# CleanDiffuserTeam/CleanDiffuser

Hardware: AMD Instinct MI355X
Metric: denoised trajectories/sec @ (B=256,H=32,D=23) 20-step DDIM (higher is better)
Workload: dtype f32; 1 GPU; BASELINE configs[1]: JannerUNet1d Diffuser H=32 D=23, 20-step DDIM, global B=256, whole DiscreteDiffusionSDE.sample() call as a pipeline makes it (initial draw inside); batch_per_gpu=256, global_batch=256, horizon=32, dim=23, sample_steps=20, world_size=1, parallelism=batch-sharded x1; the only data-path collective is the all-gather of the result

## Files before the change

### cleandiffuser_amd/csrc/cdx_unet2.hip

```cpp
#include <hip/hip_runtime.h>
#include <stdint.h>
#include <string.h>

#include "../../include/cdx.h"
#include "cdx_ops2.h"

typedef float f32x4 __attribute__((ext_vector_type(4)));
typedef const int __attribute__((address_space(4))) cint;
#pragma clang diagnostic push
#pragma clang diagnostic ignored "-Wold-style-cast"
static __device__ __forceinline__ const cint* as_const(const int* p) { return (const cint*)p; }
#pragma clang diagnostic pop

void cdx_set_err(const char* msg);

template <int NWV> struct WG {
    static constexpr int THREADS = NWV * 64;
    static constexpr int PF = NWV == 8 ? 8 : 16;
    static constexpr int OPW = CDX2_HDR_WORDS + NWV * CDX2_ITEM_WORDS;
};

namespace {

__device__ __forceinline__ float mish2(float x) {
// ... 100 lines not shown
__device__ __forceinline__ int load_desc(const int* __restrict__ ops, int op, int lane, int wave) {
    const int w = lane < CDX2_HDR_WORDS ? lane : CDX2_HDR_WORDS + wave * CDX2_ITEM_WORDS + (lane & (CDX2_ITEM_WORDS - 1));
    return ops[op * WG<NWV>::OPW + w];
}
__device__ __forceinline__ Item inline_item(int vd) {
    const int b = CDX2_HDR_WORDS;
    return make_item(CDX2_DW(vd, b + CDX2_I2_WOFF), CDX2_DW(vd, b + CDX2_I2_NQ), CDX2_DW(vd, b + CDX2_I2_TAPCC),
                     CDX2_DW(vd, b + CDX2_I2_PART), CDX2_DW(vd, b + CDX2_I2_COL0), CDX2_DW(vd, b + CDX2_I2_PADOOFF),
                     CDX2_DW(vd, b + CDX2_I2_SRCSTR), CDX2_DW(vd, b + CDX2_I2_CCN));
}

__device__ __forceinline__ void stamp(unsigned long long* slot, int tid) {
    if (slot && tid == 0) *slot = __builtin_amdgcn_s_memtime();
}

typedef unsigned u32x4 __attribute__((ext_vector_type(4)));
#ifndef CDX2_WPOLICY
#define CDX2_WPOLICY 0
#endif
#ifndef CDX2_PARAMS_ALL
#define CDX2_PARAMS_ALL 0
#endif
#define CDX2_N_CUS 256
#define CDX2_GETREG_XCC_ID ((3 << 11) | 20)
#ifndef CDX2_XCHG_FAST
#define CDX2_XCHG_FAST 1
#endif
#ifndef CDX2_XCHG_NOWAIT
#define CDX2_XCHG_NOWAIT 0
#endif
#ifndef CDX2_PROF_FETCH
#define CDX2_PROF_FETCH 0
#endif
#ifndef CDX2_PIPE_PARAMS
#define CDX2_PIPE_PARAMS 1
#endif
#ifndef CDX2_MUL24
#define CDX2_MUL24 1
#endif
static __device__ __forceinline__ int mul24i(int a, int b) { return CDX2_MUL24 ? __mul24(a, b) : a * b; }
static __device__ __forceinline__ int wave_of(int tid) { return __builtin_amdgcn_readfirstlane(tid >> 6); }
#pragma clang diagnostic push
#pragma clang diagnostic ignored "-Wold-style-cast"
struct WStream {
    __amdgpu_buffer_rsrc_t rs;
    int lane16;
    __device__ __forceinline__ WStream(const float* wblob, int lane)
        : rs(__builtin_amdgcn_make_buffer_rsrc((void*)wblob, 0, 0x7fffffff, 0x00020000)), lane16(lane * 16) {}
    __device__ __forceinline__ f32x4 load(int woff, int q) const {
        return __builtin_bit_cast(f32x4, __builtin_amdgcn_raw_buffer_load_b128(rs, lane16, woff * 4 + q * 1024, CDX2_WPOLICY));
    }
};
#pragma clang diagnostic pop

template <int PF> struct Ring { f32x4 rec[PF]; };

template <class M, int NT, int T, int NWV, bool PROF, bool GRP = false>
__device__ __forceinline__ void conv_kloop(const Geom& g, const float* __restrict__ wblob, int vd, const cint* ops,
                                           Item it, int n_items, float* __restrict__ lds, int tf, int lane, int wave,
                                           Ring<WG<NWV>::PF>& ring, unsigned long long* prof, int tune) {
    constexpr int PF = WG<NWV>::PF, NW = NWV;
    constexpr int BD = NWV == 4 ? ((M::KSTEP == 4 && NT * T == 1) ? 8 : 4)
                                : (NT * T == 1 ? (M::KSTEP == 4 ? 8 : 4) : (NT * T == 2 ? 4 : 2));
    constexpr int NA = NWV == 4 ? 4 : ((M::KSTEP == 4 && NT == 1) ? 4 : 2);
    static_assert(PF % BD == 0, "operand ring must divide the weight ring");
    const int ptid = (wave == 0 && lane == 0) ? 0 : 1;
    for (int item = wave; item < n_items; item += NW) {
        if (item != wave) it = load_item(ops + CDX2_DW(vd, CDX2_W2_ITEMS) + (item - NW) * CDX2_ITEM_WORDS);
        const int nq = it.nq, ccn = it.ccn;
        int cc = it.cc;
        int cur[NT], tstep[NT], mcol[NT];
#pragma unroll
        for (int nt = 0; nt < NT; ++nt) {
            mcol[nt] = it.col0 + nt * M::COLS + M::col(lane);
            const bool valid = mcol[nt] < g.l_cols;
            int mrow = mul24i(mcol[nt], g.cstride);
            if (GRP && g.grows) mrow = mul24i(mcol[nt] >> g.gsh, g.grows) + mul24i(mcol[nt] & ((1 << g.gsh) - 1), g.cstride);
            const int row = valid ? mrow - it.pad + CDX2_HALO2 + it.tap : 0;
            cur[nt] = it.src + __mul24(row, it.sstr) + M::koff(lane) + cc * M::KSTEP;
            tstep[nt] = (valid ? it.sstr : 0) - ccn * M::KSTEP;
        }
        if (PROF && !CDX2_PROF_FETCH && prof && item == 0) { asm volatile("" ::"s"(nq), "v"(cur[0])); stamp(prof + 4, ptid); }
        f32x4 acc[T][NT][NA];
#pragma unroll
        for (int t = 0; t < T; ++t)
#pragma unroll
            for (int nt = 0; nt < NT; ++nt)
#pragma unroll
                for (int j = 0; j < NA; ++j) acc[t][nt][j] = (f32x4){0.f, 0.f, 0.f, 0.f};

        const WStream ws(wblob, lane);
        const int woff = it.woff;
#define CDX2_WLOAD(q) ws.load(woff, (q))
// ... 79 lines not shown
#pragma unroll
                        for (int nt = 0; nt < NT; ++nt)
                            bq[ua % BD][t][nt] = *reinterpret_cast<const f32x4*>(
                                ldsb + (ua < PF ? rb[nt] : rbn[nt]) + t * tf * 4 + (ua % PF) * M::KSTEP * 4);
#pragma unroll
                    for (int j = 0; j < 4; ++j)
#pragma unroll
                        for (int t = 0; t < T; ++t)
#pragma unroll
                            for (int nt = 0; nt < NT; ++nt)
                                acc[t][nt][j % NA] = M::mfma(wr[u][j], bq[u % BD][t][nt][j], acc[t][nt][j % NA]);
                    if (u > 0) refill(u - 1, qi + u - 1 + PF);
                    else if (qi > 0) refill(PF - 1, qi - 1 + PF);
                    if (NWV == 4 || T >= 2) __builtin_amdgcn_sched_barrier(0);
                }
#pragma unroll
                for (int nt = 0; nt < NT; ++nt) rb[nt] = rbn[nt];
            }
            cc = cc0 + BD - 2;
#pragma unroll
            for (int nt = 0; nt < NT; ++nt) cur[nt] = rb[nt] / 4 + (BD - 2) * M::KSTEP;
        }
        for (; qi < nq; qi += PF) {
#pragma unroll
            for (int u = 0; u < PF; ++u) {
                if (qi + u >= nq) break;
                chunk(wr[u], u, qi + u + BD - 1 < nq);
                const int q = qi + u - 1 + PF;
                if (q >= PF && q < nq) refill((u + PF - 1) % PF, q);
            }
        }
        if (NWV == 8) __builtin_amdgcn_s_setprio(0);
        if (PROF && !CDX2_PROF_FETCH && prof && item == 0) { asm volatile("" ::"v"(acc[0][0][0][0]), "v"(acc[0][0][1][0])); stamp(prof + 6, ptid); }
#pragma unroll
        for (int t = 0; t < T; ++t)
#pragma unroll
            for (int nt = 0; nt < NT; ++nt) {
                if (mcol[nt] < g.l_cols) {
                    const int n = mul24i(mcol[nt], g.ostride) + it.ooff;
                    f32x4 dd = acc[t][nt][0];
                    if (NA == 2) dd += acc[t][nt][NA - 1];
                    if (NA == 4) dd = (acc[t][nt][0] + acc[t][nt][1]) + (acc[t][nt][NA / 2] + acc[t][nt][NA - 1]);
                    *reinterpret_cast<f32x4*>(lds + t * tf + g.stage + it.part + mul24i(n, g.sstride) + M::drow(lane)) = dd;
                }
            }
    }
}

struct EpiDesc {
    int flags, c_out, l_out, coutp, sstride, ksplit, dst, dstride, res, rstride, shift, nk;
    int save, savestr, stats, dst2, d2stride;
    int kpost;
    float inv_cnt;
    float odiv;
    int cgreal4;
};
template <bool BWD>
__device__ __forceinline__ EpiDesc decode_epi(int vd) {
    EpiDesc e;
    e.flags = CDX2_DW(vd, CDX2_W2_FLAGS); e.c_out = CDX2_DW(vd, CDX2_W2_COUT); e.l_out = CDX2_DW(vd, CDX2_W2_LOUT);
    e.coutp = CDX2_DW(vd, CDX2_W2_COUTP); e.sstride = CDX2_DW(vd, CDX2_W2_SSTRIDE); e.ksplit = CDX2_DW(vd, CDX2_W2_KSPLIT);
    e.dst = CDX2_DW(vd, CDX2_W2_DST); e.dstride = CDX2_DW(vd, CDX2_W2_DST_STRIDE); e.res = CDX2_DW(vd, CDX2_W2_RES);
    e.rstride = CDX2_DW(vd, CDX2_W2_RES_STRIDE); e.shift = CDX2_DW(vd, CDX2_W2_CG4_SHIFT); e.nk = CDX2_DW(vd, CDX2_W2_NK);
    e.inv_cnt = __int_as_float(CDX2_DW(vd, CDX2_W2_INV_CNT));
    e.kpost = CDX2_DW(vd, CDX2_W2_KPOST);
    e.odiv = BWD ? 1.0f : __int_as_float(CDX2_DW(vd, CDX2_W2_ODIV));
    e.cgreal4 = BWD ? 0 : CDX2_DW(vd, CDX2_W2_CGREAL4);
    e.save = e.savestr = e.stats = e.dst2 = e.d2stride = 0;
    if (BWD && (e.flags & (CDX2_F2_SAVE | CDX2_F2_GNBWD))) {
        e.save = CDX2_DW(vd, CDX2_W2_SAVE); e.savestr = CDX2_DW(vd, CDX2_W2_SAVE_STRIDE); e.stats = CDX2_DW(vd, CDX2_W2_STATS);
        e.dst2 = CDX2_DW(vd, CDX2_W2_DST2); e.d2stride = CDX2_DW(vd, CDX2_W2_DST2_STRIDE);
    }
    return e;
}

// ... 232 lines not shown
template <int THREADS>
__device__ __forceinline__ void run_head_fwd(const cdx_unet2_launch& L, int vd, const float* __restrict__ emb_row, float* __restrict__ tl,
                                             int tid, float* __restrict__ out) {
    const int hidden = CDX2_DW(vd, CDX2_W2_COUT), len = CDX2_DW(vd, CDX2_W2_LOUT), ch = CDX2_DW(vd, CDX2_W2_LCOLS);
    const int src = CDX2_DW(vd, CDX2_W2_RES), sstr = CDX2_DW(vd, CDX2_W2_RES_STRIDE);
    const float* __restrict__ w1 = L.wblob + CDX2_DW(vd, CDX2_W2_BOFF);
    const float* __restrict__ w2 = L.wblob + CDX2_DW(vd, CDX2_W2_GAMMA);
    const float* __restrict__ ev = emb_row + CDX2_DW(vd, CDX2_W2_EMB);
    float* hz = tl + L.stage_off;
    for (int j = tid; j < hidden; j += THREADS) {
        float z = ev[j];
        for (int l = 0; l < len; ++l) {
#pragma unroll 8
            for (int c = 0; c < ch; ++c) z = fmaf(w1[(size_t)(l * ch + c) * hidden + j], tl[src + (l + CDX2_HALO2) * sstr + c], z);
        }
        hz[j] = w2[j] * mish2(z);
    }
    __syncthreads();
    if (tid == 0 && out != nullptr) {
        float y = w2[hidden];
        for (int j = 0; j < hidden; ++j) y += hz[j];
        *out = y;
    }
    __syncthreads();
}

template <int PF>
__device__ __forceinline__ void prefetch_ring(const Item& it, const float* __restrict__ wblob, int lane, Ring<PF>& ring) {
    const WStream ws(wblob, lane);
#pragma unroll
    for (int u = 0; u < PF; ++u) ring.rec[u] = ws.load(it.woff, u);
}

template <bool COND, bool SPLIT_T, bool ALL, bool MLP = false, bool GRP = false>
__device__ __forceinline__ EpiParams load_params(const cdx_unet2_launch& L, int vd, const float* __restrict__ emb_row, int emb_tstride,
                                                 int tid, int wave, bool epi_wave) {
    const int etid = tid & 255, li = etid & 31;
    int grp = etid >> 5;
    if (GRP) {
        const int xg = CDX2_DW(vd, CDX2_W2_XG);
        if (xg & CDX2_XG_GOP) grp = (xg & 255) + (grp & ((((xg >> 8) & 255) - (xg & 255)) - 1));
    }
    const int flags = CDX2_DW(vd, CDX2_W2_FLAGS), coutp = CDX2_DW(vd, CDX2_W2_COUTP), shift = CDX2_DW(vd, CDX2_W2_CG4_SHIFT);
    const int c = mul24i(grp, coutp >> 3) + 4 * (li & ((1 << shift) - 1));
    const float* __restrict__ pbi = ((MLP && (flags & CDX2_F2_BIAS_EMB)) ? emb_row : L.wblob) + CDX2_DW(vd, CDX2_W2_BOFF) + c;
    const bool gn = (flags & (CDX2_F2_GN | CDX2_F2_GNBWD)) != 0;
    const float* __restrict__ pem = emb_row + (COND && SPLIT_T ? (wave >> 2) * emb_tstride : 0) + CDX2_DW(vd, CDX2_W2_EMB) + c;
    EpiParams P;
    if (ALL) {
        P.bi = *reinterpret_cast<const f32x4*>(pbi);
        P.pb = *reinterpret_cast<const f32x4*>(CDX2_DW(vd, CDX2_W2_KPOST) ? L.wblob + CDX2_DW(vd, CDX2_W2_PBIAS) + c : pbi);
        P.ga = *reinterpret_cast<const f32x4*>(gn ? L.wblob + CDX2_DW(vd, CDX2_W2_GAMMA) + c : pbi);
        P.be = *reinterpret_cast<const f32x4*>(gn ? L.wblob + CDX2_DW(vd, CDX2_W2_BETA) + c : pbi);
        P.em = *reinterpret_cast<const f32x4*>((flags & CDX2_F2_EMB) ? pem + ((COND && (flags & CDX2_F2_FILM)) ? coutp : 0) : pbi);
        P.sc = P.bi;
        if (COND) P.sc = *reinterpret_cast<const f32x4*>((flags & CDX2_F2_FILM) ? pem : pbi);
        return P;
    }
    P.bi = P.ga = P.be = P.em = P.pb = P.sc = (f32x4){0.f, 0.f, 0.f, 0.f};
    if (epi_wave) {
        P.bi = *reinterpret_cast<const f32x4*>(pbi);
        if (CDX2_DW(vd, CDX2_W2_KPOST)) P.pb = *reinterpret_cast<const f32x4*>(L.wblob + CDX2_DW(vd, CDX2_W2_PBIAS) + c);
        if (gn) {
            P.ga = *reinterpret_cast<const f32x4*>(L.wblob + CDX2_DW(vd, CDX2_W2_GAMMA) + c);
            P.be = *reinterpret_cast<const f32x4*>(L.wblob + CDX2_DW(vd, CDX2_W2_BETA) + c);
        }
        if (COND && (flags & CDX2_F2_FILM)) {
            P.sc = *reinterpret_cast<const f32x4*>(pem);
            P.em = *reinterpret_cast<const f32x4*>(pem + coutp);
        } else if (flags & CDX2_F2_EMB) P.em = *reinterpret_cast<const f32x4*>(pem);
    }
    return P;
}

struct OpFetch {
    EpiParams P;
    int vdn2;
};
template <int T, bool BWD> constexpr bool pipe_params() { return CDX2_PIPE_PARAMS && T < 3 && !BWD; }

struct XState {
    int m, k;
    unsigned seq;
    bool dead;
};

__device__ __forceinline__ void xchg_report(int what, const XState& X, int seq, int item, int grp) {
    const KArg* S0 = kernarg();
    asm volatile("" : "+s"(S0));
    int* e = S0->xerr;
    e[1] = what; e[2] = (int)blockIdx.x; e[3] = seq; e[4] = item;
    e[5] = (int)(__builtin_amdgcn_s_getreg(CDX2_GETREG_XCC_ID) & 15); e[6] = X.m; e[7] = grp;
// ... 97 lines not shown
        int pending = (1 << km1) - 1, spins = 0;
        while (pending) {
#pragma unroll
            for (int r = 0; r < 3; ++r) {
                if (!(pending & (1 << r))) continue;
                if (__float_as_uint(a[r][1]) == seq && __float_as_uint(a[r][3]) == seq && __float_as_uint(b[r][1]) == seq &&
                    __float_as_uint(b[r][3]) == seq) {
                    *reinterpret_cast<f32x4*>(tl + dst + row + cc[r]) = (f32x4){a[r][0], a[r][2], b[r][0], b[r][2]};
                    pending &= ~(1 << r);
                } else {
                    asm volatile("" ::: "memory");
                    const f32x4* src = reinterpret_cast<const f32x4*>(tile + (size_t)(tbase + cc[r]) * 2);
                    a[r] = __builtin_nontemporal_load(src);
                    b[r] = __builtin_nontemporal_load(src + 1);
                }
            }
            if (pending) {
                if (X.dead || ++spins > 200000) {
                    if (!X.dead) xchg_report(1, X, (int)seq, j, grp_idx);
                    X.dead = true;
                    break;
                }
                __builtin_amdgcn_s_sleep(1);
            }
        }
    }
}

template <int T, int NWV, bool BWD, bool PROF, bool COND, bool MLP = false, bool SPLIT = false, bool MEMBER = SPLIT>
__device__ __forceinline__ void run_op(const cdx_unet2_launch& L, const cint* ops, int vd, int vdn, Item& it,
                                       const float* __restrict__ emb_row, int emb_tstride, float* __restrict__ lds, int tid,
                                       Ring<WG<NWV>::PF>& ring, unsigned long long* prof, int b0, OpFetch& F,
                                       const float* __restrict__ emb_next, int emb_next_tstride, int op_next2, int pass = 0,
                                       XState* X = nullptr) {
    constexpr bool SPLIT_T = NWV == 8 && T >= 2;
    constexpr bool PIPE = pipe_params<T, BWD>();
    constexpr bool PARAMS_AFTER_BARRIER = PIPE && T >= 2;
    auto fetch_next = [&](bool params) {
        it = inline_item(vdn);
        if (PROF && CDX2_PROF_FETCH == 1) stamp(prof ? prof + 4 : nullptr, tid);
        if (wave_of(tid) < CDX2_DW(vdn, CDX2_W2_NITEMS)) prefetch_ring(it, L.wblob, tid & 63, ring);
        if (PROF && CDX2_PROF_FETCH == 1) stamp(prof ? prof + 5 : nullptr, tid);
        if (PIPE) {
            if (params)
                F.P = load_params<COND, SPLIT_T, false, MLP, MEMBER>(L, vdn, emb_next, emb_next_tstride, tid, wave_of(tid), NWV == 4 || SPLIT_T || wave_of(tid) < 4);
            if (PROF && CDX2_PROF_FETCH == 1) stamp(prof ? prof + 6 : nullptr, tid);
            F.vdn2 = load_desc<NWV>(L.ops, op_next2 + (MEMBER ? X->m * L.n_ops : 0), tid & 63, wave_of(tid));
        }
    };
    const int lane = tid & 63, wave = __builtin_amdgcn_readfirstlane(tid >> 6);
    const int tf = L.traj_floats;
    if (BWD && CDX2_DW(vd, CDX2_W2_KIND) == CDX2_KIND2_HEAD) {
        fetch_next(true);
#pragma unroll 1
        for (int t = 0; t < T; ++t) run_head<WG<NWV>::THREADS>(L, vd, emb_row, lds + t * tf, tid);
        return;
    }
    if (BWD && CDX2_DW(vd, CDX2_W2_KIND) == CDX2_KIND2_LOADX) {
        fetch_next(true);
        const int dst = CDX2_DW(vd, CDX2_W2_DST), dstr = CDX2_DW(vd, CDX2_W2_DST_STRIDE);
        const int len = CDX2_DW(vd, CDX2_W2_LOUT), ch = CDX2_DW(vd, CDX2_W2_COUT);
        const int b_end = L.traj_first + L.traj_count;
        const KArg* S = kernarg();
        asm volatile("" : "+s"(S));
#pragma unroll 1
        for (int t = 0; t < T; ++t) {
            const float* __restrict__ xg = S->x_out + (size_t)(b0 + t) * len * ch;
            const bool real = b0 + t < b_end;
            for (int i = tid; i < (len + 2 * CDX2_HALO2) * dstr; i += WG<NWV>::THREADS) {
                const int r = i / dstr, c = i - r * dstr, n = r - CDX2_HALO2;
                lds[t * tf + dst + i] = (real && n >= 0 && n < len && c < ch) ? xg[n * ch + c] : 0.f;
            }
        }
        __syncthreads();
        return;
    }
    if (MLP && CDX2_DW(vd, CDX2_W2_KIND) == CDX2_KIND2_LOADC) {
        fetch_next(true);
// ... 5 lines not shown
        asm volatile("" : "+s"(S));
        const float* __restrict__ cg = pass == 0 ? S->ctx : nullptr;
#pragma unroll 1
        for (int t = 0; t < T; ++t) {
            const bool real = cg != nullptr && b0 + t < b_end;
            const float* __restrict__ cb = cg + (size_t)(b0 + t) * len * ch;
            for (int i = tid; i < (len + 2 * CDX2_HALO2) * dstr; i += WG<NWV>::THREADS) {
                const int r = i / dstr, c = i - r * dstr, n = r - CDX2_HALO2;
                lds[t * tf + dst + i] = (real && n >= 0 && n < len && c < ch) ? cb[n * ch + c] : 0.f;
            }
        }
        __syncthreads();
        return;
    }
    const int flags = CDX2_DW(vd, CDX2_W2_FLAGS), coutp = CDX2_DW(vd, CDX2_W2_COUTP), shift = CDX2_DW(vd, CDX2_W2_CG4_SHIFT);
    const int l_out = CDX2_DW(vd, CDX2_W2_LOUT), sstride = CDX2_DW(vd, CDX2_W2_SSTRIDE);
    int gmap0 = 0;
    if (SPLIT && (CDX2_DW(vd, CDX2_W2_XG) & CDX2_XG_GOP)) gmap0 = CDX2_DW(vd, CDX2_W2_GMAP);
    const Geom g{CDX2_DW(vd, CDX2_W2_LCOLS), CDX2_DW(vd, CDX2_W2_CSTRIDE), CDX2_DW(vd, CDX2_W2_OSTRIDE), sstride, L.stage_off,
                 gmap0 & 255, gmap0 >> 8};
    const bool epi_wave = NWV == 4 || SPLIT_T || wave < 4;
    const bool halo_wave = NWV == 4 || SPLIT_T || wave >= 4;

    const int etid = tid & 255;
    const int grp = etid >> 5, li = etid & 31;
    const int c = mul24i(grp, coutp >> 3) + 4 * (li & ((1 << shift) - 1));
    const int pos0 = li >> shift, pstep = 32 >> shift;
    const int nv = (coutp >> 5) * l_out;
    EpiParams P = PIPE ? F.P : load_params<COND, SPLIT_T, CDX2_PARAMS_ALL != 0, MLP, MEMBER>(L, vd, emb_row, emb_tstride, tid, wave, epi_wave);

    const int n_items = CDX2_DW(vd, CDX2_W2_NITEMS);
    if (SPLIT && gmap0 != 0) {
        if (CDX2_DW(vd, CDX2_W2_MODE) == CDX_MODE_4X4) {
            if (CDX2_DW(vd, CDX2_W2_NT) == 1) conv_kloop<M4, 1, T, NWV, PROF, SPLIT>(g, L.wblob, vd, ops, it, n_items, lds, tf, lane, wave, ring, prof, L.tune);
            else conv_kloop<M4, 2, T, NWV, PROF, SPLIT>(g, L.wblob, vd, ops, it, n_items, lds, tf, lane, wave, ring, prof, L.tune);
        } else {
            conv_kloop<M16, 1, T, NWV, PROF, SPLIT>(g, L.wblob, vd, ops, it, n_items, lds, tf, lane, wave, ring, prof, L.tune);
        }
    } else if (CDX2_DW(vd, CDX2_W2_MODE) == CDX_MODE_4X4) {
        if (CDX2_DW(vd, CDX2_W2_NT) == 1) conv_kloop<M4, 1, T, NWV, PROF>(g, L.wblob, vd, ops, it, n_items, lds, tf, lane, wave, ring, prof, L.tune);
        else conv_kloop<M4, 2, T, NWV, PROF>(g, L.wblob, vd, ops, it, n_items, lds, tf, lane, wave, ring, prof, L.tune);
    } else {
        conv_kloop<M16, 1, T, NWV, PROF>(g, L.wblob, vd, ops, it, n_items, lds, tf, lane, wave, ring, prof, L.tune);
    }
    if (PROF) stamp(prof ? prof + 7 : nullptr, tid);
    fetch_next(!PARAMS_AFTER_BARRIER);
    if (PROF) stamp(prof ? prof + 1 : nullptr, tid);
    __syncthreads();
    if (PROF) stamp(prof ? prof + 2 : nullptr, tid);
    const EpiParams Pnext = PARAMS_AFTER_BARRIER ? load_params<COND, SPLIT_T, false, MLP, MEMBER>(L, vdn, emb_next, emb_next_tstride, tid, wave, epi_wave)
                                                 : (PIPE ? F.P : P);

    const EpiDesc e = decode_epi<BWD>(vd);
    int xgw = 0, gmap = 0;
    if (SPLIT) {
        int vde = vd;
        asm volatile("" : "+v"(vde));
        xgw = CDX2_DW(vde, CDX2_W2_XG);
        if (BWD && (e.flags & (CDX2_F2_SAVE | CDX2_F2_GNBWD | CDX2_F2_DUAL))) xgw = 0;
        if (xgw & (CDX2_XG_GOP | CDX2_XG_TRAJ)) gmap = CDX2_DW(vde, CDX2_W2_GMAP);
    }
    if (SPLIT && (xgw & CDX2_XG_GOP)) {
        const int gx_lo = xgw & 255, gpm = ((xgw >> 8) & 255) - gx_lo, grows = gmap >> 8;
        const bool xfast = CDX2_XCHG_FAST && (xgw & CDX2_XG_XCHG) != 0;
        const unsigned xseq = X->seq + 1;
        float* xtile = xfast ? exchange_tile(*X, xseq, __float_as_int(lds[T * tf])) : nullptr;
        if (epi_wave) {
            const int g_t = __builtin_amdgcn_readfirstlane(gpm == 4 ? grp >> 2 : grp >> 1);
            const int cgo = mul24i(gx_lo + (grp & (gpm - 1)), coutp >> 3) + 4 * (li & ((1 << shift) - 1));
            EpiDesc eg = e;
            eg.dst += g_t * grows * e.dstride;
            eg.res += g_t * grows * e.rstride;
            eg.l_out = l_out * X->k;
            const int stage_g = g.stage + g_t * l_out * sstride - gx_lo * (coutp >> 3);
            bool withhold = false;
            if (xfast) {
                const KArg* S0 = kernarg();
                asm volatile("" : "+s"(S0));
                withhold = S0->fault != 0 && X->m == S0->fault - 1;
            }
            const Pub pub{xtile, __uint_as_float(xseq), g_t * l_out, e.coutp, xfast && !withhold};
            if (e.nk == 1) epilogue<1, BWD, COND, MLP, true>(lds, P, eg, stage_g, cgo, pos0, pstep, li, nv, lane, grp, nullptr, &pub);
            else epilogue<2, BWD, COND, MLP, true>(lds, P, eg, stage_g, cgo, pos0, pstep, li, nv, lane, grp, nullptr, &pub);
// ... 149 lines not shown
    __syncthreads();
    auto logp_only_f = [&]() -> bool {
        if (!BWD) return false;
        const KArg* S0 = kernarg();
        asm volatile("" : "+s"(S0));
        return S0->n_steps == 0 && S0->logp_out != nullptr;
    };
    const int n_iter = logp_only_f() ? 0 : (L.n_steps > 0 ? L.n_steps : 1);
    const int HDp = (HD + 3) & ~3;
    constexpr bool PIPE = pipe_params<T, BWD>();
    constexpr bool SPLIT_T0 = NWV == 8 && T >= 2;
    int n_pass_all = 1;
    if (COND) {
        const KArg* S0 = kernarg();
        asm volatile("" : "+s"(S0));
        n_pass_all = S0->n_pass == 2 ? 2 : 1;
    }
    auto emb_of = [&](int step, int pass, int& tstride) -> const float* {
        const float* row = L.emb + (size_t)step * L.emb_ld;
        tstride = 0;
        if (COND) {
            const KArg* S0 = kernarg();
            asm volatile("" : "+s"(S0));
            if (pass == 1) row = S0->emb_u + (size_t)step * L.emb_ld;
            else if (S0->emb_per_traj) {
                row = L.emb + ((size_t)step * L.batch + b0) * L.emb_ld;
                tstride = L.emb_ld;
            }
        }
        return row;
    };
    OpFetch F;
    int vdn_keep = 0;
    if (PIPE) {
        int ts0;
        const float* row0 = emb_of(0, 0, ts0);
        F.P = load_params<COND, SPLIT_T0, false, MLP>(L, vd, row0, ts0, tid, wave, NWV == 4 || SPLIT_T0 || wave < 4);
        vdn_keep = load_desc<NWV>(L.ops, moff + (L.n_ops > 1 ? 1 : 0), lane, wave);
    }
    for (int step = 0; step < n_iter; ++step) {
      const int n_pass = n_pass_all;
#pragma unroll 1
      for (int pass = 0; pass < n_pass; ++pass) {
        int emb_tstride, emb_next_tstride;
        const float* __restrict__ emb_row = emb_of(step, pass, emb_tstride);
        const bool last_fwd = pass + 1 == n_pass && step + 1 >= n_iter;
        const float* __restrict__ emb_fwd_next = last_fwd ? emb_of(step, pass, emb_next_tstride)
                                                          : emb_of(pass + 1 < n_pass ? step : step + 1, pass + 1 < n_pass ? pass + 1 : 0, emb_next_tstride);
        const int ts_fwd_next = emb_next_tstride;
        for (int oi = 0; oi < L.n_ops; ++oi) {
            const int vdn = PIPE ? vdn_keep : load_desc<NWV>(L.ops, moff + (oi + 1 < L.n_ops ? oi + 1 : 0), lane, wave);
            unsigned long long* pslot = (profiling && step == (L.n_steps > 1 ? 1 : 0)) ? lprof + (size_t)oi * 8 : nullptr;
            if (PROF) stamp(pslot, tid);
            const bool wrap = oi + 1 >= L.n_ops;
            int on2 = oi + 2;
            if (on2 >= L.n_ops) on2 -= L.n_ops;
            if (on2 >= L.n_ops) on2 = 0;
            run_op<T, NWV, BWD, PROF, COND, MLP, SPLIT, SPLIT>(L, ops, vd, vdn, it, emb_row, emb_tstride, lds, tid, ring, pslot, b0, F,
                                                               wrap ? emb_fwd_next : emb_row, wrap ? ts_fwd_next : emb_tstride, on2,
                                                               (MLP && n_pass == 1 && step > 0) ? 2 : pass, &X);
            vd = vdn;
            if (PIPE) vdn_keep = F.vdn2;
        }
        if (COND && n_pass == 2 && pass == 0) {
            const KArg* S = kernarg();
            asm volatile("" : "+s"(S));
#pragma unroll 1
            for (int t = 0; t < T; ++t) {
                if (b0 + t >= b_end) break;
                const size_t xbase = (size_t)(b0 + t) * HD;
                float* tl = lds + t * tf;
                float* wsb = S->ws + (size_t)(b0 + t) * S->ws_floats;
                const float c_in = S->edm_plan ? S->steps[step].alpha : 1.0f;
                for (int e = tid; e < HD; e += THREADS) {
                    const int n = e / D, c = e - n * D;
                    wsb[2 * HDp + e] = tl[S->pred_off + n * S->pred_stride + c];
                    if (S->compact) tl[S->x_off + n * S->x_stride + c] = c_in * S->x_out[xbase + e];
                }
                if (S->compact) {
                    const int xs = S->x_stride, xb = S->x_off - CDX2_HALO2 * xs;
                    for (int i = tid; i < (H + 2 * CDX2_HALO2) * xs; i += THREADS) {
                        const int r = i / xs, c = i - r * xs;
                        if (r < CDX2_HALO2 || r >= H + CDX2_HALO2 || c >= D) tl[xb + i] = 0.f;
                    }
                }
            }
            __syncthreads();
        }
      }
        if (L.n_steps == 0) break;
        const KArg* S = kernarg();
        asm volatile("" : "+s"(S));
        const cdx_step st = S->steps[step];
        const float al = st.alpha, sg = st.sigma;
        const float k0 = st.k[0], k1 = st.k[1], k2 = st.k[2], k3 = st.k[3], k4 = st.k[4];
        const bool edm = COND && st.kind >= 5;
        const bool xglob = S->compact || edm;
        const float c_next = (edm && step + 1 < S->n_steps) ? S->steps[step + 1].alpha : 1.0f;
#pragma unroll 1
        for (int t = 0; t < T; ++t) {
            if (b0 + t >= b_end) break;
            const int b = b0 + t;
            const size_t xbase = (size_t)b * HD;
            float* tl = lds + t * tf;
            float* wsb = (COND && (xglob || n_pass == 2)) ? S->ws + (size_t)b * S->ws_floats : nullptr;
            for (int e = tid; e < HD; e += THREADS) {
                const int n = e / D, c = e - n * D;
                const int xo = S->x_off + n * S->x_stride + c;
                const float x = xglob ? S->x_out[xbase + e] : tl[xo];
                float p = tl[S->pred_off + n * S->pred_stride + c];
                if (COND && n_pass == 2) p = S->cfg_w * wsb[2 * HDp + e] + (1.0f - S->cfg_w) * p;
                if (edm) {
                    float dn = k0 * x + k1 * p, xe;
                    if (S->x_min) dn = fmaxf(dn, S->x_min[e]);
                    if (S->x_max) dn = fminf(dn, S->x_max[e]);
                    if (st.kind == 7) {
                        xe = dn;
                        if (S->fix_mask) {
                            const float m = S->fix_mask[e];
                            xe = xe * (1.0f - m) + S->prior[xbase + e] * m;
                        }
                        if (st.noise_idx >= 0) xe += k3 * S->noise[((size_t)st.noise_idx * S->batch + b) * HD + e];
                    } else {
// ... 44 lines not shown
                    xn = k0 * ((x - k1 * eps) / k2) + k3 * eps;
                } else {
                    if (st.flags & CDX_STEP_MASK_PRED) {
                        const float m = S->fix_mask ? S->fix_mask[e] : 0.f;
                        eps = eps * (1.0f - m);
                        xth = xth * (1.0f - m) + x * m;
                    }
                    float v = (st.vsel & 1) ? xth : eps;
                    if (st.vsel == 2) v = k3 * xth - k4 * (S->compact ? S->ws[(size_t)b * S->ws_floats + e] : tl[S->prev_off + e]);
                    if (st.vsel == 3) v = k3 * eps - k4 * (S->compact ? S->ws[(size_t)b * S->ws_floats + e] : tl[S->prev_off + e]);
                    xn = k0 * x - k1 * v;
                    if (st.noise_idx >= 0) xn += k2 * S->noise[((size_t)st.noise_idx * S->batch + b) * HD + e];
                }
                if (S->fix_mask) {
                    const float m = S->fix_mask[e];
                    xn = xn * (1.0f - m) + S->prior[xbase + e] * m;
                }
                if (st.push) {
                    if (S->compact) S->ws[(size_t)b * S->ws_floats + e] = st.push == 2 ? eps : xth;
                    else tl[S->prev_off + e] = st.push == 2 ? eps : xth;
                }
                tl[xo] = xn;
                if (S->compact) S->x_out[xbase + e] = xn;
            }
            if (S->compact) {
                const int xs = S->x_stride, xb = S->x_off - CDX2_HALO2 * xs;
                for (int i = tid; i < (H + 2 * CDX2_HALO2) * xs; i += THREADS) {
                    const int r = i / xs, c = i - r * xs;
                    if (r < CDX2_HALO2 || r >= H + CDX2_HALO2 || c >= D) tl[xb + i] = 0.f;
                }
            }
        }
        __syncthreads();
    }
    const bool logp_only = logp_only_f();
    if (BWD && (L.n_steps > 0 || logp_only)) {
        const KArg* S = kernarg();
        asm volatile("" : "+s"(S));
        if (S->logp_out != nullptr) {
            const int first = S->logp_first_op, head = S->logp_head_op;
            const float* __restrict__ emb_row = L.emb + (size_t)(logp_only ? b0 : L.n_steps) * L.emb_ld;
            vd = load_desc<NWV>(L.ops, moff + first, lane, wave);
            it = inline_item(vd);
            if (wave < CDX2_DW(vd, CDX2_W2_NITEMS)) prefetch_ring(it, L.wblob, lane, ring);
            for (int oi = first; oi < head; ++oi) {
                const int vdn = load_desc<NWV>(L.ops, moff + oi + 1, lane, wave);
                run_op<T, NWV, BWD, PROF, COND>(L, ops, vd, vdn, it, emb_row, 0, lds, tid, ring, nullptr, b0, F, emb_row, 0, 0);
                vd = vdn;
            }
#pragma unroll 1
            for (int t = 0; t < T; ++t)
                run_head_fwd<THREADS>(L, vd, emb_row, lds + t * tf, tid, b0 + t < b_end ? S->logp_out + (b0 + t) : nullptr);
        }
    }
#pragma unroll 1
    for (int t = 0; t < T; ++t) {
        if (b0 + t >= b_end) break;
        const size_t xbase = (size_t)(b0 + t) * HD;
        const KArg* S = kernarg();
        asm volatile("" : "+s"(S));
        const bool want_grad = BWD && S->n_steps == 0 && S->grad_off >= 0 && S->with_backward;
        const int off = S->n_steps == 0 ? (want_grad ? S->grad_off : S->pred_off) : S->x_off;
        const int str = S->n_steps == 0 ? (want_grad ? S->grad_stride : S->pred_stride) : S->x_stride;
        float* __restrict__ xo = S->x_out;
        if ((S->compact || (COND && S->edm_plan)) && S->n_steps > 0) break;
        const bool poisoned = SPLIT && __syncthreads_or(X.dead ? 1 : 0) != 0;
        if (SPLIT && !grouped && X.m != 0) break;
        if (BWD && logp_only) break;
        for (int e = tid; e < HD; e += THREADS) {
            const int n = e / D, c = e - n * D;
            xo[xbase + e] = (SPLIT && poisoned) ? __builtin_nanf("") : lds[t * tf + off + n * str + c];
        }
    }
    if (profiling) {
        stamp(lprof + (size_t)L.n_ops * 8 + 1, tid);
        __syncthreads();
        for (int i = tid; i < L.n_ops * 8 + 2; i += THREADS) L.prof[i] = lprof[i];
    }
}

__global__ __launch_bounds__(256) void cdx_unet2_embtab_kernel(const cdx_unet2_embtab_args A) {
    extern __shared__ __attribute__((aligned(16))) float sh[];
    float* v0 = sh;
    float* h = v0 + A.emb_dim;
    float* m = h + A.hidden;
    float* raw = m + A.md;
    const int r = blockIdx.x, tid = threadIdx.x;
    for (int i = tid; i < A.emb_dim; i += 256) v0[i] = A.temb[(size_t)r * A.emb_dim + i];
    __syncthreads();
    for (int o = tid; o < A.hidden; o += 256) {
        float acc = A.wblob[A.b0 + o];
        for (int i = 0; i < A.emb_dim; ++i) acc = fmaf(A.wblob[A.w0 + (size_t)i * A.hidden + o], v0[i], acc);
        h[o] = mish2(acc);
    }
    __syncthreads();
    for (int o = tid; o < A.md; o += 256) {
        float acc = A.wblob[A.b2 + o];
        for (int i = 0; i < A.hidden; ++i) acc = fmaf(A.wblob[A.w2 + (size_t)i * A.md + o], h[i], acc);
        raw[o] = acc;
        m[o] = mish2(acc);
    }
    __syncthreads();
    float* orow = A.out + (size_t)r * A.out_ld;
    for (int o = tid; o < A.n_emb; o += 256) {
        float acc = A.wblob[A.b3 + o];
        for (int i = 0; i < A.md; ++i) acc = fmaf(A.wblob[A.w3 + (size_t)i * A.n_emb + o], m[i], acc);
        orow[A.col0 + o] = acc;
    }
// ... 131 lines not shown
```

### cleandiffuser_amd/engine/runtime2.py

```python
import ctypes
import os
import warnings
import weakref
from typing import NamedTuple, Optional

import torch

from . import program2 as P2
from . import runtime as R


class CdxUnet2EmbtabArgs(ctypes.Structure):
    _fields_ = [("wblob", ctypes.c_void_p),
                ("emb_dim", ctypes.c_int32), ("hidden", ctypes.c_int32), ("md", ctypes.c_int32), ("n_emb", ctypes.c_int32),
                ("w0", ctypes.c_int32), ("b0", ctypes.c_int32), ("w2", ctypes.c_int32), ("b2", ctypes.c_int32),
                ("w3", ctypes.c_int32), ("b3", ctypes.c_int32),
                ("temb", ctypes.c_void_p), ("n_rows", ctypes.c_int32), ("out", ctypes.c_void_p),
                ("out_ld", ctypes.c_int32), ("col0", ctypes.c_int32),
                ("w4", ctypes.c_int32), ("b4", ctypes.c_int32), ("n_raw", ctypes.c_int32), ("col4", ctypes.c_int32)]


class CdxUnet2Launch(ctypes.Structure):
    _fields_ = [("ops", ctypes.c_void_p), ("wblob", ctypes.c_void_p),
                ("n_ops", ctypes.c_int32), ("traj_floats", ctypes.c_int32), ("traj_per_wg", ctypes.c_int32),
# ... 610 lines not shown
        k = group_factor(batch) if group else split_factor(batch)
        if k > 1:
            if guided:
                comp = (compiled_guided_group2 if group else compiled_guided_split2)(net, clf_net, horizon, k)
            else:
                comp = (compiled_group2 if group else compiled_split2)(net, horizon, k)
            return Route("grouped" if group else "split", k, comp, guided) if comp.prog is not None else None
    return None


def _launch_members(dev, route: Route, member_kw: dict, plain: _Compiled2, kw: dict, outs: dict, **plain_kw) -> dict:
    launch(route.comp, split=route.k, group=route.group, t_per_wg=1, **member_kw, **outs)
    launch(plain, run_if=_split_err(dev), **plain_kw, **kw, **outs)
    ok = _MODE_FLAGS[route.group, route.guided]
    if dev in ok:
        return outs
    ref = {name: torch.empty_like(t) for name, t in outs.items()}
    launch(plain, **plain_kw, **kw, **ref)
    try:
        check_split_errors(dev, wait=True)
        good = all(bool(torch.allclose(outs[name], ref[name], rtol=1e-3, atol=1e-3)) for name in outs)
    except RuntimeError as e:
        warnings.warn(f"first-use check of the {'grouped' if route.group else 'small-batch'}{' guided' if route.guided else ''} mode: {e}")
        good = False
    ok[dev] = good
    return outs if good else ref


def stream_bytes_per_forward(prog: P2.Program2, member: int = 0) -> int:
    ops = prog.meta["member_ops"][member] if "member_ops" in prog.meta else prog.ops
    return 1024 * sum(int(P2.op_item(prog.ops_buffer, op, j)[P2.I2_NQ]) for op in ops for j in range(int(op[P2.W2_NITEMS])))


def route_info(net, horizon: int, batch: int, device) -> dict:
    comp, parts = plan_for(net, horizon, batch)
    route = None if comp.prog.compact else member_route(net, horizon, batch, torch.device(device), capturing=False)
    if route is None:
        mode, k, n_wg = "plain", 1, sum(-(-cnt // t) for _, cnt, t in parts)
    else:
        mode, k, comp, parts, n_wg = route.mode, route.k, route.comp, None, N_CUS
    return {"mode": mode, "k": k, "comp": comp, "parts": parts, "workgroups": n_wg,
            "stream_bytes_per_workgroup_forward": stream_bytes_per_forward(comp.prog)}


def backbone_forward2(module, x, noise_t, condition=None) -> Optional[torch.Tensor]:
    b, h, d = x.shape
    if supported(module, h) is not None:
        return None
    if b == 0:
        return torch.empty_like(R._f32c(x, x.device))
    comp, t_wg = shape_for(module, h, b)
    if comp.prog.compact:
        return None
    chi = R._is_chiunet(module)
    if chi:
        if condition is None:
            return None
        condition = torch.flatten(condition, 1)
        if tuple(condition.shape) != (b, comp.prog.meta["cond_dim"]):
            return None
    elif condition is not None and (condition.dim() != 2 or tuple(condition.shape) != (b, comp.prog.emb_dim)):
        return None
    with torch.no_grad():
        t = noise_t.reshape(-1)
        if t.shape[0] == 1:
            t = t.expand(b)
        if chi:
            emb = chi_film_table(comp, module, t.contiguous(), R._f32c(condition, x.device), per_sample=True)
        else:
            emb = cond_film_table(comp, module, t.contiguous(), None if condition is None else R._f32c(condition, x.device), per_sample=True)
        xin = R._f32c(x, x.device)
        out = torch.empty_like(xin)
        launch(comp, batch=b, x_in=xin, x_out=out, emb=emb, t_per_wg=t_wg, emb_per_traj=True)
    return out

# ... 233 lines not shown
```

Baseline: 70670 trajectories/s.

## Store plain conv outputs directly with bias, skipping staging and epilogue pass

For simple 16x16 conv ops that have no GN, embedding, k-split or post ops and whose item count fits the waves, the k-loop now adds the bias and writes results straight into the destination activation buffer in LDS. The halo rows are zeroed separately, and the op returns after a single barrier, skipping the staging write and the separate epilogue pass with its params and descriptor decode. The path is gated by a tune bit that is off by default, and the host reports which ops qualify. It also adds an optional per-step profiling stamp. The extra branches in the k-loop and param loading add code size and may raise register pressure.

```diff
diff --git a/cleandiffuser_amd/csrc/cdx_unet2.hip b/cleandiffuser_amd/csrc/cdx_unet2.hip
--- a/cleandiffuser_amd/csrc/cdx_unet2.hip
+++ b/cleandiffuser_amd/csrc/cdx_unet2.hip
@@ -156,6 +156,9 @@
 #ifndef CDX2_PROF_FETCH
 #define CDX2_PROF_FETCH 0
 #endif
+#ifndef CDX2_PROF_STEP
+#define CDX2_PROF_STEP 0
+#endif
 #ifndef CDX2_PIPE_PARAMS
 #define CDX2_PIPE_PARAMS 1
 #endif
@@ -177,12 +180,22 @@
 };
 #pragma clang diagnostic pop
 
+template <int NWV>
+__device__ __forceinline__ bool direct_store_op(int vd, int vtune) {
+    if (CDX2_DW(vd, CDX2_W2_FLAGS) & ~CDX2_F2_PRED) return false;
+    if (CDX2_DW(vd, CDX2_W2_KIND) != CDX2_KIND2_CONV || CDX2_DW(vd, CDX2_W2_MODE) != CDX_MODE_16X16) return false;
+    if (CDX2_DW(vd, CDX2_W2_KSPLIT) != 1 || CDX2_DW(vd, CDX2_W2_KPOST) != 0 || CDX2_DW(vd, CDX2_W2_XG) != 0) return false;
+    if (CDX2_DW(vd, CDX2_W2_NITEMS) > NWV) return false;
+    return (__builtin_amdgcn_readfirstlane(vtune) & 1) == 0;
+}
+
 template <int PF> struct Ring { f32x4 rec[PF]; };
 
-template <class M, int NT, int T, int NWV, bool PROF, bool GRP = false>
+template <class M, int NT, int T, int NWV, bool PROF, bool GRP = false, bool DS = false>
 __device__ __forceinline__ void conv_kloop(const Geom& g, const float* __restrict__ wblob, int vd, const cint* ops,
                                            Item it, int n_items, float* __restrict__ lds, int tf, int lane, int wave,
-                                           Ring<WG<NWV>::PF>& ring, unsigned long long* prof, int tune) {
+                                           Ring<WG<NWV>::PF>& ring, unsigned long long* prof, int vtune,
+                                           const f32x4& bias = f32x4{0.f, 0.f, 0.f, 0.f}) {
     constexpr int PF = WG<NWV>::PF, NW = NWV;
     constexpr int BD = NWV == 4 ? ((M::KSTEP == 4 && NT * T == 1) ? 8 : 4)
                                 : (NT * T == 1 ? (M::KSTEP == 4 ? 8 : 4) : (NT * T == 2 ? 4 : 2));
@@ -328,6 +341,12 @@
         }
         if (NWV == 8) __builtin_amdgcn_s_setprio(0);
         if (PROF && !CDX2_PROF_FETCH && prof && item == 0) { asm volatile("" ::"v"(acc[0][0][0][0]), "v"(acc[0][0][1][0])); stamp(prof + 6, ptid); }
+        bool direct = false;
+        int d_dst = 0, d_stride = 0, d_cout = 0;
+        if (DS && direct_store_op<NWV>(vd, vtune)) {
+            direct = true;
+            d_dst = CDX2_DW(vd, CDX2_W2_DST); d_stride = CDX2_DW(vd, CDX2_W2_DST_STRIDE); d_cout = CDX2_DW(vd, CDX2_W2_COUT);
+        }
 #pragma unroll
         for (int t = 0; t < T; ++t)
 #pragma unroll
@@ -337,6 +356,19 @@
                     f32x4 dd = acc[t][nt][0];
                     if (NA == 2) dd += acc[t][nt][NA - 1];
                     if (NA == 4) dd = (acc[t][nt][0] + acc[t][nt][1]) + (acc[t][nt][NA / 2] + acc[t][nt][NA - 1]);
+                    if (DS && direct) {
+                        const int c = it.part + M::drow(lane);
+                        f32x4 y = bias;
+                        y += dd;
+                        float* o = lds + t * tf + d_dst + mul24i(n + CDX2_HALO2, d_stride) + c;
+                        if (c + 3 < d_cout) {
+                            *reinterpret_cast<f32x4*>(o) = y;
+                        } else {
+#pragma unroll
+                            for (int j = 0; j < 4; ++j)
+                                if (c + j < d_cout) o[j] = y[j];
+                        }
+                    } else
                     *reinterpret_cast<f32x4*>(lds + t * tf + g.stage + it.part + mul24i(n, g.sstride) + M::drow(lane)) = dd;
                 }
             }
@@ -635,9 +667,9 @@
     for (int u = 0; u < PF; ++u) ring.rec[u] = ws.load(it.woff, u);
 }
 
-template <bool COND, bool SPLIT_T, bool ALL, bool MLP = false, bool GRP = false>
+template <bool COND, bool SPLIT_T, bool ALL, bool MLP = false, bool GRP = false, int DSNW = 0>
 __device__ __forceinline__ EpiParams load_params(const cdx_unet2_launch& L, int vd, const float* __restrict__ emb_row, int emb_tstride,
-                                                 int tid, int wave, bool epi_wave) {
+                                                 int tid, int wave, bool epi_wave, int vtune = 0) {
     const int etid = tid & 255, li = etid & 31;
     int grp = etid >> 5;
     if (GRP) {
@@ -661,6 +693,11 @@
         return P;
     }
     P.bi = P.ga = P.be = P.em = P.pb = P.sc = (f32x4){0.f, 0.f, 0.f, 0.f};
+    if (DSNW != 0 && direct_store_op<(DSNW ? DSNW : 4)>(vd, vtune)) {
+        if (wave < CDX2_DW(vd, CDX2_W2_NITEMS))
+            P.bi = *reinterpret_cast<const f32x4*>(L.wblob + CDX2_DW(vd, CDX2_W2_BOFF) + CDX2_DW(vd, CDX2_HDR_WORDS + CDX2_I2_PART) + M16::drow(tid & 63));
+        return P;
+    }
     if (epi_wave) {
         P.bi = *reinterpret_cast<const f32x4*>(pbi);
         if (CDX2_DW(vd, CDX2_W2_KPOST)) P.pb = *reinterpret_cast<const f32x4*>(L.wblob + CDX2_DW(vd, CDX2_W2_PBIAS) + c);
@@ -824,9 +861,11 @@
                                        const float* __restrict__ emb_row, int emb_tstride, float* __restrict__ lds, int tid,
                                        Ring<WG<NWV>::PF>& ring, unsigned long long* prof, int b0, OpFetch& F,
                                        const float* __restrict__ emb_next, int emb_next_tstride, int op_next2, int pass = 0,
-                                       XState* X = nullptr) {
+                                       XState* X = nullptr, int vtune = 1) {
     constexpr bool SPLIT_T = NWV == 8 && T >= 2;
     constexpr bool PIPE = pipe_params<T, BWD>();
+    constexpr bool DSTORE = PIPE && !BWD && !COND && !MLP;
+    constexpr int DSNW = DSTORE ? NWV : 0;
     constexpr bool PARAMS_AFTER_BARRIER = PIPE && T >= 2;
     auto fetch_next = [&](bool params) {
         it = inline_item(vdn);
@@ -835,7 +874,7 @@
         if (PROF && CDX2_PROF_FETCH == 1) stamp(prof ? prof + 5 : nullptr, tid);
         if (PIPE) {
             if (params)
-                F.P = load_params<COND, SPLIT_T, false, MLP, MEMBER>(L, vdn, emb_next, emb_next_tstride, tid, wave_of(tid), NWV == 4 || SPLIT_T || wave_of(tid) < 4);
+                F.P = load_params<COND, SPLIT_T, false, MLP, MEMBER, DSNW>(L, vdn, emb_next, emb_next_tstride, tid, wave_of(tid), NWV == 4 || SPLIT_T || wave_of(tid) < 4, vtune);
             if (PROF && CDX2_PROF_FETCH == 1) stamp(prof ? prof + 6 : nullptr, tid);
             F.vdn2 = load_desc<NWV>(L.ops, op_next2 + (MEMBER ? X->m * L.n_ops : 0), tid & 63, wave_of(tid));
         }
@@ -907,23 +946,40 @@
     const int n_items = CDX2_DW(vd, CDX2_W2_NITEMS);
     if (SPLIT && gmap0 != 0) {
         if (CDX2_DW(vd, CDX2_W2_MODE) == CDX_MODE_4X4) {
-            if (CDX2_DW(vd, CDX2_W2_NT) == 1) conv_kloop<M4, 1, T, NWV, PROF, SPLIT>(g, L.wblob, vd, ops, it, n_items, lds, tf, lane, wave, ring, prof, L.tune);
-            else conv_kloop<M4, 2, T, NWV, PROF, SPLIT>(g, L.wblob, vd, ops, it, n_items, lds, tf, lane, wave, ring, prof, L.tune);
+            if (CDX2_DW(vd, CDX2_W2_NT) == 1) conv_kloop<M4, 1, T, NWV, PROF, SPLIT>(g, L.wblob, vd, ops, it, n_items, lds, tf, lane, wave, ring, prof, 1);
+            else conv_kloop<M4, 2, T, NWV, PROF, SPLIT>(g, L.wblob, vd, ops, it, n_items, lds, tf, lane, wave, ring, prof, 1);
         } else {
-            conv_kloop<M16, 1, T, NWV, PROF, SPLIT>(g, L.wblob, vd, ops, it, n_items, lds, tf, lane, wave, ring, prof, L.tune);
+            conv_kloop<M16, 1, T, NWV, PROF, SPLIT>(g, L.wblob, vd, ops, it, n_items, lds, tf, lane, wave, ring, prof, 1);
         }
     } else if (CDX2_DW(vd, CDX2_W2_MODE) == CDX_MODE_4X4) {
-        if (CDX2_DW(vd, CDX2_W2_NT) == 1) conv_kloop<M4, 1, T, NWV, PROF>(g, L.wblob, vd, ops, it, n_items, lds, tf, lane, wave, ring, prof, L.tune);
-        else conv_kloop<M4, 2, T, NWV, PROF>(g, L.wblob, vd, ops, it, n_items, lds, tf, lane, wave, ring, prof, L.tune);
+        if (CDX2_DW(vd, CDX2_W2_NT) == 1) conv_kloop<M4, 1, T, NWV, PROF>(g, L.wblob, vd, ops, it, n_items, lds, tf, lane, wave, ring, prof, 1);
+        else conv_kloop<M4, 2, T, NWV, PROF>(g, L.wblob, vd, ops, it, n_items, lds, tf, lane, wave, ring, prof, 1);
     } else {
-        conv_kloop<M16, 1, T, NWV, PROF>(g, L.wblob, vd, ops, it, n_items, lds, tf, lane, wave, ring, prof, L.tune);
+        conv_kloop<M16, 1, T, NWV, PROF, false, DSTORE>(g, L.wblob, vd, ops, it, n_items, lds, tf, lane, wave, ring, prof, vtune, P.bi);
     }
     if (PROF) stamp(prof ? prof + 7 : nullptr, tid);
     fetch_next(!PARAMS_AFTER_BARRIER);
     if (PROF) stamp(prof ? prof + 1 : nullptr, tid);
+    if (DSTORE && direct_store_op<NWV>(vd, vtune)) {
+        if (PROF) stamp(prof ? prof + 2 : nullptr, tid);
+        if (PARAMS_AFTER_BARRIER) F.P = load_params<COND, SPLIT_T, false, MLP, MEMBER, DSNW>(L, vdn, emb_next, emb_next_tstride, tid, wave, epi_wave, vtune);
+        if (halo_wave) {
+            const int dst = CDX2_DW(vd, CDX2_W2_DST), dstride = CDX2_DW(vd, CDX2_W2_DST_STRIDE);
+            const int hw = wave & 3;
+            const int hrow = hw < CDX2_HALO2 ? hw : l_out + hw;
+            const int t_lo = SPLIT_T ? (wave >> 2) : 0, t_step = SPLIT_T ? 2 : 1;
+#pragma unroll 1
+            for (int t = t_lo; t < T; t += t_step)
+                for (int j = lane * 4; j < dstride; j += 256)
+                    *reinterpret_cast<f32x4*>(lds + t * tf + dst + hrow * dstride + j) = (f32x4){0.f, 0.f, 0.f, 0.f};
+        }
+        __syncthreads();
+        if (PROF) stamp(prof ? prof + 3 : nullptr, tid);
+        return;
+    }
     __syncthreads();
     if (PROF) stamp(prof ? prof + 2 : nullptr, tid);
-    const EpiParams Pnext = PARAMS_AFTER_BARRIER ? load_params<COND, SPLIT_T, false, MLP, MEMBER>(L, vdn, emb_next, emb_next_tstride, tid, wave, epi_wave)
+    const EpiParams Pnext = PARAMS_AFTER_BARRIER ? load_params<COND, SPLIT_T, false, MLP, MEMBER, DSNW>(L, vdn, emb_next, emb_next_tstride, tid, wave, epi_wave, vtune)
                                                  : (PIPE ? F.P : P);
 
     const EpiDesc e = decode_epi<BWD>(vd);
@@ -1139,10 +1195,12 @@
     };
     OpFetch F;
     int vdn_keep = 0;
+    int vtune = L.tune;
+    asm volatile("" : "+v"(vtune));
     if (PIPE) {
         int ts0;
         const float* row0 = emb_of(0, 0, ts0);
-        F.P = load_params<COND, SPLIT_T0, false, MLP>(L, vd, row0, ts0, tid, wave, NWV == 4 || SPLIT_T0 || wave < 4);
+        F.P = load_params<COND, SPLIT_T0, false, MLP, false, (!BWD && !COND && !MLP) ? NWV : 0>(L, vd, row0, ts0, tid, wave, NWV == 4 || SPLIT_T0 || wave < 4, vtune);
         vdn_keep = load_desc<NWV>(L.ops, moff + (L.n_ops > 1 ? 1 : 0), lane, wave);
     }
     for (int step = 0; step < n_iter; ++step) {
@@ -1165,7 +1223,7 @@
             if (on2 >= L.n_ops) on2 = 0;
             run_op<T, NWV, BWD, PROF, COND, MLP, SPLIT, SPLIT>(L, ops, vd, vdn, it, emb_row, emb_tstride, lds, tid, ring, pslot, b0, F,
                                                                wrap ? emb_fwd_next : emb_row, wrap ? ts_fwd_next : emb_tstride, on2,
-                                                               (MLP && n_pass == 1 && step > 0) ? 2 : pass, &X);
+                                                               (MLP && n_pass == 1 && step > 0) ? 2 : pass, &X, vtune);
             vd = vdn;
             if (PIPE) vdn_keep = F.vdn2;
         }
@@ -1196,6 +1254,8 @@
         }
       }
         if (L.n_steps == 0) break;
+        const bool prof_step = PROF && CDX2_PROF_STEP && profiling && step == (L.n_steps > 1 ? 1 : 0);
+        if (prof_step) stamp(lprof + (size_t)L.n_ops * 8, tid);
         const KArg* S = kernarg();
         asm volatile("" : "+s"(S));
         const cdx_step st = S->steps[step];
@@ -1306,6 +1366,7 @@
             }
         }
         __syncthreads();
+        if (prof_step) stamp(lprof + (size_t)L.n_ops * 8 + 1, tid);
     }
     const bool logp_only = logp_only_f();
     if (BWD && (L.n_steps > 0 || logp_only)) {
@@ -1347,7 +1408,7 @@
         }
     }
     if (profiling) {
-        stamp(lprof + (size_t)L.n_ops * 8 + 1, tid);
+        if (!CDX2_PROF_STEP) stamp(lprof + (size_t)L.n_ops * 8 + 1, tid);
         __syncthreads();
         for (int i = tid; i < L.n_ops * 8 + 2; i += THREADS) L.prof[i] = lprof[i];
     }
diff --git a/cleandiffuser_amd/engine/runtime2.py b/cleandiffuser_amd/engine/runtime2.py
--- a/cleandiffuser_amd/engine/runtime2.py
+++ b/cleandiffuser_amd/engine/runtime2.py
@@ -666,6 +666,20 @@
     return 1024 * sum(int(P2.op_item(prog.ops_buffer, op, j)[P2.I2_NQ]) for op in ops for j in range(int(op[P2.W2_NITEMS])))
 
 
+def direct_store_ops(prog: P2.Program2) -> list:
+    if prog is None or any(k in prog.meta for k in ("mlp", "chi_film", "head_op")) or prog.grad_off >= 0:
+        return []
+    if int(os.environ.get("CDX_UNET2_TUNE", DEFAULT_TUNE)) & 1:
+        return []
+
+    def ok(op) -> bool:
+        return (int(op[P2.W2_KIND]) == P2.KIND2_CONV and int(op[P2.W2_MODE]) == P2.MODE_16X16 and int(op[P2.W2_KSPLIT]) == 1
+                and int(op[P2.W2_KPOST]) == 0 and (int(op[P2.W2_FLAGS]) & ~P2.F2_PRED) == 0 and int(op[P2.W2_XG]) == 0
+                and int(op[P2.W2_NITEMS]) <= prog.nw)
+    views = prog.meta.get("member_ops", [prog.ops])
+    return [i for i in range(len(prog.ops)) if all(ok(v[i]) for v in views)]
+
+
 def route_info(net, horizon: int, batch: int, device) -> dict:
     comp, parts = plan_for(net, horizon, batch)
     route = None if comp.prog.compact else member_route(net, horizon, batch, torch.device(device), capturing=False)
@@ -673,8 +687,9 @@
         mode, k, n_wg = "plain", 1, sum(-(-cnt // t) for _, cnt, t in parts)
     else:
         mode, k, comp, parts, n_wg = route.mode, route.k, route.comp, None, N_CUS
+    direct = [] if (parts is not None and any(t == 3 for _, _, t in parts)) else direct_store_ops(comp.prog)
     return {"mode": mode, "k": k, "comp": comp, "parts": parts, "workgroups": n_wg,
-            "stream_bytes_per_workgroup_forward": stream_bytes_per_forward(comp.prog)}
+            "stream_bytes_per_workgroup_forward": stream_bytes_per_forward(comp.prog), "direct_store_ops": direct}
 
 
 def backbone_forward2(module, x, noise_t, condition=None) -> Optional[torch.Tensor]:
```

New measurement: 66900 trajectories/s. -5.3%, worse.
